# Wangshihu12/Voxel-SLAM

Measured on AMD Instinct MI355X. Metric: local-BA iterations/sec (200k pts, W=10), higher is better.
Workload: dtype f64

## Files before the change

### voxel-slam_amd/csrc/vba_kernels_li.hpp

```cpp
#pragma once
#include <hip/hip_runtime.h>
#include "vba_hostmath.hpp"
#include "vba_li_order.hpp"

namespace vba {

constexpr int LI_MAX_W = 16;
constexpr int LI_MAX_N = 15 * LI_MAX_W + 3;

struct LiDev {
  int W, n, nb, gravity, gauge, F;
  double imu_coef;
  double ex[LI_MAX_W * 12];
  double ext[LI_MAX_W * 12];
  double tstamp[LI_MAX_W];
  double rimu[2];
  double ext_spec[LM_SPEC][LI_MAX_W * 12];
  double ginc_spec[LM_SPEC][4];
  double binc_spec[LM_SPEC][LI_MAX_W * 6];
};

__device__ __forceinline__ void li_state(const double *pose12, const double *ex12, double t, vbh::State &s) {
  s.t = t;
#pragma unroll
// ... 332 lines not shown
  if (tid < F) {
    vbh::State s1, s2;
    li_state(s->xt + 12 * tid, li->ext + 12 * tid, li->tstamp[tid], s1);
    li_state(s->xt + 12 * (tid + 1), li->ext + 12 * (tid + 1), li->tstamp[tid + 1], s2);
    double rr[15];
    vbh::imu_residual_jacobian(*reinterpret_cast<const vbh::ImuPre *>(imu + 304 * (size_t)tid), s1, s2, li->gravity != 0, rr, nullptr, li->nb);
    for (int k = 0; k < 15; k++) rr_s[tid][k] = rr[k];
  }
  __syncthreads();
  if (tid < 15 * F) {
    const int f = tid / 15, r = tid - 15 * f;
    const double *m = imu + 304 * (size_t)f + 79 + 15 * r;
    double a = 0;
    for (int k = 0; k < 15; k++) a += m[k] * rr_s[f][k];
    a_s[f][r] = a;
  }
  __syncthreads();
  if (tid >= 64) return;
  double qi = 0.0;
  if (lane < F) for (int r = 0; r < 15; r++) qi += rr_s[lane][r] * a_s[lane][r];
  double rimu = 0.0;
  for (int f = 0; f < F; f++) rimu += readlane_f64(qi, f);
  double r2;
  if (nb > 0) {
    double acc = r2acc;
    for (int m = 32; m >= 1; m >>= 1) acc += __shfl_xor(acc, m, 64);
    r2 = acc;
  } else {
    r2 = readlane_f64(r2acc, 0);
  }
  r2 += rimu * (li->imu_coef * 0.5);
  const bool have_spec = spec_nx < spec_n;
  const int sc = have_spec ? spec_nx : 0;
  double q = r1 - r2, u = u0, v = v0;
  const bool accept = q > 0;
  if (accept) {
    for (int t = lane; t < 12 * W; t += 64) { s->x[t] = s->xt[t]; li->ex[t] = li->ext[t]; }
    const double one_three = 1.0 / 3;
    q = q / q1;
    v = 2;
    const double t = 2 * q - 1;
    q = 1 - t * t * t;
    u *= (q < one_three ? one_three : q);
  } else {
    u = u * v;
    v = 2 * v;
    if (lane < F) { double *m = imu + 304 * (size_t)lane; for (int k = 0; k < 3; k++) { m[67 + k] = m[73 + k]; m[70 + k] = m[76 + k]; } }
    if (have_spec) {
      double gn[3] = {0, 0, 0};
      if (li->gravity) for (int k = 0; k < 3; k++) gn[k] = li->ext[9 + k] + li->ginc_spec[sc][k];
      for (int t = lane; t < 12 * W; t += 64) {
        s->xt[t] = s->xt_spec[sc][t];
        const int k = t % 12;
        if (k < 9) li->ext[t] = li->ext_spec[sc][t];
        else if (li->gravity) li->ext[t] = gn[k - 9];
      }
      if (lane < F) {
        double *m = imu + 304 * (size_t)lane;
        for (int k = 0; k < 6; k++) m[67 + k] = m[73 + k] + li->binc_spec[sc][6 * lane + k];
      }
    }
  }
  if (lane != 0) return;
  if (!accept && have_spec) { s->q1 = s->q1_spec[sc]; s->spec_i = sc; s->use_spec = 1; }
  else { s->use_spec = 0; s->spec_n = 0; }
  li->rimu[1] = rimu;
  s->r2 = r2;
  if (ntr < mtr) {
    double *t = s->trace + 5 * ntr;
    t[0] = r1; t[1] = r2; t[2] = u0; t[3] = v0; t[4] = q1;
    s->n_trace = ntr + 1;
  }
  s->u = u; s->v = v;
  s->is_calc_hess = accept ? 1 : 0;
  s->last_accepted = accept ? 1 : 0;
  if (!accept) s->all_accepted = 0;
  s->iter = it + 1;
  const int nstop = (fabs((r1 - r2) / r1) < 1e-6) ? 1 : 0;
  s->stop = nstop;
  s->run_res = nstop ? 0 : 1;
  s->run_hess = (accept && !nstop) ? 1 : 0;
}

struct PackSegs { int n; const double *src[8]; size_t off[8], len[8]; };
__global__ void k_pack_segments(PackSegs p, double *__restrict__ dst) {
  const int s = blockIdx.y;
  if (s >= p.n) return;
  const double *src = p.src[s];
  double *d = dst + p.off[s];
  for (size_t i = (size_t)blockIdx.x * blockDim.x + threadIdx.x; i < p.len[s]; i += (size_t)gridDim.x * blockDim.x) d[i] = src[i];
}

}
```

### voxel-slam_amd/csrc/vba_li_order.hpp

```cpp
#pragma once

#if defined(__HIPCC__)
#include <hip/hip_runtime.h>
#define LIO_HD __host__ __device__ inline
#else
#define LIO_HD inline
#endif

namespace vba {

LIO_HD int li_ord(int k, int W) {
  if (k < 9 * W) { const int i = k / 9; return 15 * i + 6 + (k - 9 * i); }
  if (k < 15 * W) { const int q = k - 9 * W, i = q / 6; return 15 * i + (q - 6 * i); }
  return k;
}

LIO_HD unsigned li_live(int kb, int W, int n, int NP) {
  const int c0 = 8 * kb, c1 = c0 + 7;
  auto span = [](int a, int b) -> unsigned { return (a < b) ? ((2u << ((b - 1) >> 4)) - 1u) & ~((1u << (a >> 4)) - 1u) : 0u; };
  if (c0 >= 9 * W) return span(c0, NP);
  const int ihi = (c1 < 9 * W ? c1 : 9 * W - 1) / 9;
  unsigned m = span(c0, (9 * (ihi + 2) < 9 * W) ? 9 * (ihi + 2) : 9 * W);
  m |= span(9 * W, (6 * (ihi + 2) < 6 * W) ? 9 * W + 6 * (ihi + 2) : 15 * W);
  m |= span(15 * W, n + 1);
  if (c1 >= 9 * W) m |= span(9 * W, NP);
  return m;
}

LIO_HD int li_hb_pair(int a, int b) { return (3 * a + (b - a)) * 225; }
LIO_HD int li_hb_ne1(int W) { return (3 * W - 2) * 225; }
LIO_HD int li_hb_size(int W, int grav) { return li_hb_ne1(W) + (grav ? 90 * W + 9 : 0); }
LIO_HD double li_hb_get(const double *hb, int W, int n, int R, int C) {
  const int nw = 15 * W;
  if (R < nw && C < nw) { const int a = R / 15, b = C / 15; if (a - b > 1 || b - a > 1) return 0.0; return hb[li_hb_pair(a, b) + (R - 15 * a) * 15 + (C - 15 * b)]; }
  const int ne1 = li_hb_ne1(W);
  if (R < nw) return hb[ne1 + R * 3 + (C - nw)];
  if (C < nw) return hb[ne1 + 45 * W + (R - nw) * nw + C];
  return hb[ne1 + 90 * W + (R - nw) * 3 + (C - nw)];
}

}

#undef LIO_HD
```

### voxel-slam_amd/csrc/voxelba.hip

```cpp
#include "vba_ctx.hpp"
#include "vba_kernels_factor.hpp"
#include "vba_kernels_h3.hpp"
#include "vba_kernels_lm.hpp"
#include "vba_kernels_li.hpp"
#include <cstddef>
#include "vba_hostmath.hpp"

#include <hip/hip_runtime.h>
#include <rccl/rccl.h>
#include <dlfcn.h>
#include <cstdio>
#include <cstdlib>
#include <cstring>
#include <string>
#include <vector>
#include <array>
#include <map>
#include <chrono>
#include <algorithm>

using namespace vba;

namespace {

// ... 733 lines not shown
    return VBA_OK;
  }
  double *h_hess = nullptr;
  if (hess) {
    st = ensure_pin(c, 65536 + (size_t)n * n + 1024);
    if (st) return st;
    h_hess = c->h_pin + 32768;
  }
  const double *src = c->collective() ? c->d_raw : c->d_out;
  const int upd = c->lm.pending_update ? 1 : 0;
  switch (W) {
#define VBA_FIN_CASE(WW) case WW: hipLaunchKernelGGL(k_lm_finish<WW>, dim3(hess ? 17 : 1), dim3(256), 0, c->stream, c->d_lm, c->d_k4part, upd ? c->lm.k4_nb : 0, upd, c->h_lm, src, h_hess); break;
    VBA_FIN_CASE(2) VBA_FIN_CASE(3) VBA_FIN_CASE(4) VBA_FIN_CASE(5) VBA_FIN_CASE(6) VBA_FIN_CASE(7) VBA_FIN_CASE(8) VBA_FIN_CASE(9) VBA_FIN_CASE(10)
    VBA_FIN_CASE(11) VBA_FIN_CASE(12) VBA_FIN_CASE(13) VBA_FIN_CASE(14) VBA_FIN_CASE(15) VBA_FIN_CASE(16)
#undef VBA_FIN_CASE
    default: return VBA_ERR_UNSUPPORTED_WINDOW;
  }
  c->lm.pending_update = false;
  HIPCHK(c, hipGetLastError());
  HIPCHK(c, hipStreamSynchronize(c->stream));
  const LmDev *h = c->h_lm;
  if (poses) std::memcpy(poses, h->x, (size_t)W * 12 * sizeof(double));
  if (hess) std::memcpy(hess, c->h_pin + 32768, (size_t)n * n * sizeof(double));
  if (resis2) { resis2[0] = h->resis_first; resis2[1] = h->r2; }
  c->trace.assign(h->trace, h->trace + 5 * h->n_trace);
  if (h->pad & 16) {
    fprintf(stderr, "[k_lm_solve_m cycles] prologue %lld | tile load %lld | factorisation %lld | backsub %lld | epilogue %lld | panels:", h->stamps[1] - h->stamps[0],
            h->stamps[2] - h->stamps[1], h->stamps[3] - h->stamps[2], h->stamps[4] - h->stamps[3], h->stamps[5] - h->stamps[4]);
    const int npr = (int)h->stamps[6];
    for (int kb = 0; kb < npr && kb < 8; kb++) fprintf(stderr, " %lld+%lld", h->stamps[9 + 2 * kb] - h->stamps[8 + 2 * kb], kb < npr - 1 ? h->stamps[10 + 2 * kb] - h->stamps[9 + 2 * kb] : 0LL);
    fprintf(stderr, " | %d panels run\n", npr);
  }
  c->lm.active = false;
  return VBA_OK;
}

int vba_lidar_ba_damping_iter(vba_ctx *c, double *poses, double *hess, double *resis2, int max_iter, int thd_num, int *is_converge) {
  int st = vba_lm_begin(c, poses, thd_num);
  if (st) return st;
  for (int i = 0; i < max_iter; i++) {
    st = vba_lm_iterate(c, nullptr, nullptr);
    if (st) { c->lm.active = false; return st; }
  }
  st = vba_lm_end(c, poses, hess, resis2);
  if (is_converge) *is_converge = c->h_lm->all_accepted;
  return st;
}

int vba_last_lm_trace(vba_ctx *c, double *rows, int max_rows) {
  int n = (int)(c->trace.size() / 5);
  if (n > max_rows) n = max_rows;
  if (rows) std::memcpy(rows, c->trace.data(), (size_t)n * 5 * sizeof(double));
  return n;
}

extern "C++" {
template <int W>
struct LiSolveCfg {
  static constexpr int NMAX = 15 * W + 3, NP = ((NMAX + 1 + 15) / 16) * 16;
  static constexpr bool GL = W > 10;
  static constexpr size_t l_doubles = (size_t)LdltCfg<NP>::LTOT > (size_t)NMAX * (NMAX + 1) / 2 ? (size_t)LdltCfg<NP>::LTOT : (size_t)NMAX * (NMAX + 1) / 2;
  static constexpr size_t lds = ((GL ? (size_t)LdltCfg<NP>::DOUBLES - LdltCfg<NP>::LTOT : (size_t)LdltCfg<NP>::DOUBLES) + 4 * NMAX + NP + 32) * 8 + (size_t)NMAX * 4 + 64;
  static_assert(GL || l_doubles == (size_t)LdltCfg<NP>::LTOT, "the staged triangle must fit the region of L");
};
template <int W, int NT = (W > 10 ? 1024 : 512)>
static int launch_li_solve(vba_ctx *c, int copy_raw, int n, int gauge, int grav) {
  constexpr bool GL = LiSolveCfg<W>::GL;
  constexpr size_t l_doubles = LiSolveCfg<W>::l_doubles, lds = LiSolveCfg<W>::lds;
  static bool attr_set[kMaxDevices] = {false};
  if (!attr_set[c->device % kMaxDevices]) { hipFuncSetAttribute((const void *)k_li_solve<W, NT, GL>, hipFuncAttributeMaxDynamicSharedMemorySize, (int)lds); attr_set[c->device % kMaxDevices] = true; }
  if (GL && c->d_liscr.n < l_doubles * LM_SPEC) {
    HIPCHK(c, hipStreamSynchronize(c->stream));
    HIPCHK(c, c->d_liscr.ensure(l_doubles * LM_SPEC));
  }
  hipLaunchKernelGGL((k_li_solve<W, NT, GL>), dim3(c->lm_spec), dim3(NT), lds, c->stream, c->d_lm, c->d_li, c->d_out, c->d_raw, copy_raw, c->d_himu, c->d_gimu, c->d_imu, n, gauge, grav,
                     c->opt.imu_coef, c->d_liscr, nullptr);
  return VBA_OK;
}
namespace vba {
bool li_device_supported(int W) { return W >= 2 && W <= LI_MAX_W; }
}
}

static int li_setup(vba_ctx *c, const double *states, const double *imus, int gravity, LiDev &h, std::vector<double> &fimg) {
  const int W = c->opt.win_size, DIM = VBA_DIM, F = W - 1;
  const int n = W * DIM + (gravity ? 3 : 0), nb = gravity ? 33 : 30;
  if (!c->d_li) {
    HIPCHK(c, c->d_li.ensure(1));
    HIPCHK(c, c->d_imu.ensure((size_t)LI_MAX_W * 304));
    HIPCHK(c, c->d_himu.ensure((size_t)LI_MAX_N * LI_MAX_N));
    HIPCHK(c, c->d_gimu.ensure((size_t)LI_MAX_N));
  }
  std::vector<double> poses((size_t)W * 12);
  states_to_poses(states, W, poses.data());
  int st = vba_lm_begin(c, poses.data(), 0);
  if (st) return st;
  st = lm_init_flush(c);
  if (st) return st;
  h = LiDev{};
  h.W = W; h.n = n; h.nb = nb; h.gravity = gravity ? 1 : 0; h.gauge = gravity ? 6 : DIM; h.F = F; h.imu_coef = c->opt.imu_coef;
  for (int i = 0; i < W; i++) {
    const double *sx = states + 25 * i;
    h.tstamp[i] = sx[0];
    for (int k = 0; k < 12; k++) h.ex[12 * i + k] = h.ext[12 * i + k] = sx[13 + k];
  }
  fimg.resize((size_t)F * 304);
  std::memcpy(fimg.data(), imus, fimg.size() * sizeof(double));
  for (int f = 0; f < F; f++) {
    const double *cov = imus + 304 * (size_t)f + 79;
    double *dst = fimg.data() + 304 * (size_t)f + 79;
    bool hit = false;
    for (auto &e : c->covinv_cache)
      if (std::memcmp(e.data(), cov, 225 * sizeof(double)) == 0) { std::memcpy(dst, e.data() + 225, 225 * sizeof(double)); hit = true; break; }
    if (!hit) {
      vbh::inverse_pplu(cov, dst, 15);
      const bool grow = c->covinv_cache.size() < 32;
      if (grow) c->covinv_cache.emplace_back();
      auto &e = grow ? c->covinv_cache.back() : c->covinv_cache[c->covinv_next++ % 32];
      std::memcpy(e.data(), cov, 225 * sizeof(double)); std::memcpy(e.data() + 225, dst, 225 * sizeof(double));
    }
  }
  {
    HIPCHK(c, hipMemcpyAsync(c->d_li, &h, sizeof(LiDev), hipMemcpyHostToDevice, c->stream));
    HIPCHK(c, hipMemcpyAsync(c->d_imu, fimg.data(), fimg.size() * sizeof(double), hipMemcpyHostToDevice, c->stream));
  }
  HIPCHK(c, hipMemsetAsync(c->d_himu, 0, (size_t)li_hb_size(W, 1) * sizeof(double), c->stream));
  HIPCHK(c, hipMemsetAsync(c->d_gimu, 0, (size_t)n * sizeof(double), c->stream));
  {
    static bool attr_set[kMaxDevices] = {false};
    constexpr int FM = LI_MAX_W - 1;
    if (!attr_set[c->device % kMaxDevices]) { hipFuncSetAttribute((const void *)k_li_imu, hipFuncAttributeMaxDynamicSharedMemorySize, (int)(((size_t)2 * FM * 15 * 33 + 2 * FM * 15 + FM + 16) * sizeof(double))); attr_set[c->device % kMaxDevices] = true; }
  }
  return VBA_OK;
}
static size_t li_imu_lds(int F, int nb) { return ((size_t)2 * F * 15 * nb + 2 * F * 15 + F + 16) * sizeof(double); }
static bool li_imu_rides(const vba_ctx *c, int copy_raw, int V, size_t lds_imu) { return !(copy_raw && c->lm.have_hess) && V > 0 && lds_imu <= 150 * 1024; }

static int li_ba_device(vba_ctx *c, double *states, double *imus, int gravity, int max_iter, double *hess, double *resis2) {
  static const bool want_times = diag_env("VBA_LI_TIMES") != nullptr;
  const auto t_0 = std::chrono::steady_clock::now();
  auto since = [&](std::chrono::steady_clock::time_point a) { return std::chrono::duration<double, std::micro>(std::chrono::steady_clock::now() - a).count(); };
  const int W = c->opt.win_size, V = c->nvox, DIM = VBA_DIM, F = W - 1;
  const int n = W * DIM + (gravity ? 3 : 0), nb = gravity ? 33 : 30, n6 = 6 * W;
  if (!gravity) max_iter = 3;
  LiDev h{};
  std::vector<double> fimg;
  int st = li_setup(c, states, imus, gravity, h, fimg);
  if (st) return st;
  char *base = reinterpret_cast<char *>(c->d_lm.p);
  const double *x_dev = reinterpret_cast<const double *>(base + offsetof(LmDev, x));
  const double *xt_dev = reinterpret_cast<const double *>(base + offsetof(LmDev, xt));
  const int *run_hess = reinterpret_cast<const int *>(base + offsetof(LmDev, run_hess));
  const int *run_res = reinterpret_cast<const int *>(base + offsetof(LmDev, run_res));
  const int copy_raw = c->collective() ? 1 : 0;
  const size_t lds_imu = li_imu_lds(F, nb);
  const double t_up = since(t_0);
  for (int it = 0; it < max_iter; it++) {
    const bool lidar_now = li_imu_rides(c, copy_raw, V, lds_imu);
    if (lidar_now) {
      const LiJob job{c->d_lm, c->d_li, c->d_imu, c->d_himu, c->d_gimu};
      st = hessian_pass(c, x_dev, run_hess, 0, V, nullptr, nullptr, 0, job, lds_imu);
    } else {
      hipLaunchKernelGGL(k_li_imu, dim3(1), dim3(LI_IMU_NT), lds_imu, c->stream, c->d_lm, c->d_li, c->d_imu, c->d_himu, c->d_gimu);
      if (!(copy_raw && c->lm.have_hess)) st = hessian_pass(c, x_dev, run_hess, 0, V);
    }
    if (st) { c->lm.active = false; return st; }
    TimedSpan s1{};
    span_begin(c, "solve", s1);
    switch (W) {
      case 2: st = launch_li_solve<2>(c, copy_raw, n, h.gauge, h.gravity); break;
      case 3: st = launch_li_solve<3>(c, copy_raw, n, h.gauge, h.gravity); break;
      case 4: st = launch_li_solve<4>(c, copy_raw, n, h.gauge, h.gravity); break;
      case 5: st = launch_li_solve<5>(c, copy_raw, n, h.gauge, h.gravity); break;
      case 6: st = launch_li_solve<6>(c, copy_raw, n, h.gauge, h.gravity); break;
      case 7: st = launch_li_solve<7>(c, copy_raw, n, h.gauge, h.gravity); break;
      case 9: st = launch_li_solve<9>(c, copy_raw, n, h.gauge, h.gravity); break;
      case 8: st = launch_li_solve<8>(c, copy_raw, n, h.gauge, h.gravity); break;
      case 10: {
        static const int nt = diag_env("VBA_LI_NT") ? atoi(diag_env("VBA_LI_NT")) : 512;
        if (nt == 256) st = launch_li_solve<10, 256>(c, copy_raw, n, h.gauge, h.gravity); else if (nt == 1024) st = launch_li_solve<10, 1024>(c, copy_raw, n, h.gauge, h.gravity); else st = launch_li_solve<10, 512>(c, copy_raw, n, h.gauge, h.gravity);
        break;
      }
      case 11: st = launch_li_solve<11>(c, copy_raw, n, h.gauge, h.gravity); break;
      case 12: st = launch_li_solve<12>(c, copy_raw, n, h.gauge, h.gravity); break;
      case 13: st = launch_li_solve<13>(c, copy_raw, n, h.gauge, h.gravity); break;
      case 14: st = launch_li_solve<14>(c, copy_raw, n, h.gauge, h.gravity); break;
      case 15: st = launch_li_solve<15>(c, copy_raw, n, h.gauge, h.gravity); break;
      case 16: st = launch_li_solve<16>(c, copy_raw, n, h.gauge, h.gravity); break;
      default: c->lm.active = false; return VBA_ERR_UNSUPPORTED_WINDOW;
    }
    span_end(c, "solve", s1);
    if (st) { c->lm.active = false; return st; }
    if (copy_raw) {
      if (V > 0) launch_residual(c, xt_dev, run_res, 0, V);
      st = hessian_pass(c, xt_dev, run_res, 0, V);
      if (st) { c->lm.active = false; return st; }
      c->lm.have_hess = true;
      hipLaunchKernelGGL(k_li_update, dim3(1), dim3(LI_UPD_NT), 0, c->stream, c->d_lm, c->d_li, c->d_imu, c->d_out + (nout_tl(W) - 1), 0);
    } else if (V == 0) {
      st = residual_pass(c, xt_dev, run_res, 0, V, c->d_scal);
      if (st) { c->lm.active = false; return st; }
      hipLaunchKernelGGL(k_li_update, dim3(1), dim3(LI_UPD_NT), 0, c->stream, c->d_lm, c->d_li, c->d_imu, c->d_scal, 0);
    } else {
      const int nbk = residual_nb(c, V);
      TimedSpan s2{};
      span_begin(c, "residual", s2);
      launch_residual(c, xt_dev, run_res, 0, V);
      span_end(c, "residual", s2);
      hipLaunchKernelGGL(k_li_update, dim3(1), dim3(LI_UPD_NT), 0, c->stream, c->d_lm, c->d_li, c->d_imu, c->d_partial, nbk);
    }
    HIPCHK(c, hipGetLastError());
  }
  const double t_enq = since(t_0);
  const double t_gpu = since(t_0);
  static_assert(sizeof(LiDev) % 8 == 0 && sizeof(LmDev) % 8 == 0, "packed as doubles");
  const size_t o_li = 0, o_img = o_li + sizeof(LiDev) / 8, o_hb = o_img + fimg.size(), o_lid = o_hb + (size_t)li_hb_size(W, 1),
               o_lm = o_lid + (size_t)n6 * n6, o_end = o_lm + sizeof(LmDev) / 8;
  st = ensure_pin(c, o_end + 64);
  if (st) return st;
  HIPCHK(c, c->d_lipack.ensure(o_end + 64));
  PackSegs segs{};
  segs.n = 3;
  segs.src[0] = (const double *)c->d_li.p; segs.off[0] = o_li; segs.len[0] = sizeof(LiDev) / 8;
  segs.src[1] = c->d_imu; segs.off[1] = o_img; segs.len[1] = fimg.size();
  segs.src[2] = (const double *)c->d_lm.p; segs.off[2] = o_lm; segs.len[2] = sizeof(LmDev) / 8;
  if (hess) {
    st = tiles_to_full(c, copy_raw ? c->d_raw : c->d_out);
    if (st) return st;
    segs.n = 5;
    segs.src[3] = c->d_full; segs.off[3] = o_lid; segs.len[3] = (size_t)n6 * n6;
    segs.src[4] = c->d_himu; segs.off[4] = o_hb; segs.len[4] = (size_t)li_hb_size(W, gravity);
  }
  hipLaunchKernelGGL(k_pack_segments, dim3(64, segs.n), dim3(256), 0, c->stream, segs, c->d_lipack);
  HIPCHK(c, hipGetLastError());
  HIPCHK(c, hipMemcpyAsync(c->h_pin, c->d_lipack, o_end * sizeof(double), hipMemcpyDeviceToHost, c->stream));
  HIPCHK(c, hipStreamSynchronize(c->stream));
  std::memcpy(c->h_lm, c->h_pin + o_lm, sizeof(LmDev));
  std::memcpy(&h, c->h_pin + o_li, sizeof(LiDev));
  std::memcpy(fimg.data(), c->h_pin + o_img, fimg.size() * sizeof(double));
  const double *himu_h = c->h_pin + o_hb;
  c->lm.active = false;
  const LmDev *hl = c->h_lm;
  for (int i = 0; i < W; i++) {
    double *sx = states + 25 * i;
    for (int k = 0; k < 12; k++) sx[1 + k] = hl->x[12 * i + k];
    for (int k = 0; k < 12; k++) sx[13 + k] = h.ex[12 * i + k];
  }
  if (hl->use_spec)
    for (int f = 0; f < F; f++) std::memcpy(fimg.data() + 304 * (size_t)f + 67, fimg.data() + 304 * (size_t)f + 73, 6 * sizeof(double));
  for (int f = 0; f < F; f++) std::memcpy(imus + 304 * (size_t)f + 67, fimg.data() + 304 * (size_t)f + 67, 12 * sizeof(double));
  if (hess) {
    const double *lid = c->h_pin + o_lid;
    for (int r = 0; r < n; r++)
      for (int k = 0; k < n; k++) hess[(size_t)r * n + k] = c->opt.imu_coef * li_hb_get(himu_h, W, n, r, k);
    for (int i = 0; i < W; i++)
      for (int j = 0; j < W; j++)
        for (int r = 0; r < 6; r++)
          for (int k = 0; k < 6; k++) hess[(size_t)(i * DIM + r) * n + j * DIM + k] += lid[(size_t)(i * 6 + r) * n6 + j * 6 + k];
  }
  if (gravity && resis2) { resis2[0] = hl->resis_first; resis2[1] = hl->r2; }
  c->trace.assign(hl->trace, hl->trace + 5 * hl->n_trace);
  if (want_times && (hl->pad & 16)) {
    fprintf(stderr, "[k_li_solve prologue] stage imu %lld | stage lidar %lld | diag+g %lld | rank %lld\n", hl->stamps[50] - hl->stamps[0], hl->stamps[51] - hl->stamps[50], hl->stamps[52] - hl->stamps[51], hl->stamps[1] - hl->stamps[52]);
    fprintf(stderr, "[k_li_solve cycles] prologue %lld | tile load %lld | factorisation %lld | backsub %lld | epilogue %lld | panels:", hl->stamps[1] - hl->stamps[0],
            hl->stamps[2] - hl->stamps[1], hl->stamps[3] - hl->stamps[2], hl->stamps[4] - hl->stamps[3], hl->stamps[5] - hl->stamps[4]);
    const int npr = (int)hl->stamps[6];
    for (int kb = 0; kb < npr && kb < 20; kb++) fprintf(stderr, " %lld+%lld", hl->stamps[9 + 2 * kb] - hl->stamps[8 + 2 * kb], kb < npr - 1 ? hl->stamps[10 + 2 * kb] - hl->stamps[9 + 2 * kb] : 0LL);
    fprintf(stderr, " | %d panels run\n", npr);
  }
  if (want_times && (hl->pad & 64)) fprintf(stderr, "[k_li_imu cycles] factor algebra (one lane per factor) %lld | cov^-1 joc %lld | contractions %lld\n", hl->stamps[41] - hl->stamps[40], hl->stamps[42] - hl->stamps[41], hl->stamps[43] - hl->stamps[42]);
  if (want_times && (hl->pad & 32)) { double v[6]; std::memcpy(v, &hl->stamps[58], sizeof(v)); fprintf(stderr, "[li r1 parts] rank %d: rimu %.10g lidar %.10g | %.10g %.10g | %.10g %.10g\n", c->rank, v[0], v[1], v[2], v[3], v[4], v[5]); }
  if (want_times) fprintf(stderr, "[li_ba_device] upload %.1f us | enqueue %.1f | gpu drained at %.1f | total %.1f\n", t_up, t_enq - t_up, t_gpu, since(t_0));
  return VBA_OK;
}

int vba_li_ba_damping_iter(vba_ctx *c, double *states, double *imus, int gravity, int max_iter, double *hess, double *resis2) {
  if (!li_device_supported(c->opt.win_size)) return VBA_ERR_UNSUPPORTED_WINDOW;
  return li_ba_device(c, states, imus, gravity, max_iter, hess, resis2);
}

static int debug_li_imu_run(vba_ctx *c, int gravity, int flags, const double *states, const double *imus, double *h_dense, double *g, double *rimu,
                            double *covinv_out) {
  const int W = c->opt.win_size, V = c->nvox, F = W - 1, n = 15 * W + (gravity ? 3 : 0), nb = gravity ? 33 : 30;
  LiDev h{};
  std::vector<double> fimg;
  int st = li_setup(c, states, imus, gravity, h, fimg);
  if (st) return st;
  char *base = reinterpret_cast<char *>(c->d_lm.p);
  const double *x_dev = reinterpret_cast<const double *>(base + offsetof(LmDev, x));
  const int *run_hess = reinterpret_cast<const int *>(base + offsetof(LmDev, run_hess));
  const size_t lds_imu = li_imu_lds(F, nb);
  if (flags & (VBA_IMU_RIDE_H2 | VBA_IMU_RIDE_H3)) {
    const LiJob job{c->d_lm, c->d_li, c->d_imu, c->d_himu, c->d_gimu};
    st = hessian_pass(c, x_dev, run_hess, 0, V, nullptr, nullptr, 0, job, lds_imu);
    if (st) return st;
  } else {
    hipLaunchKernelGGL(k_li_imu, dim3(1), dim3(LI_IMU_NT), lds_imu, c->stream, c->d_lm, c->d_li, c->d_imu, c->d_himu, c->d_gimu);
  }
  HIPCHK(c, hipGetLastError());
  if (flags & VBA_IMU_TRIAL) {
    HIPCHK(c, hipMemsetAsync(c->d_scal, 0, sizeof(double), c->stream));
    hipLaunchKernelGGL(k_li_update, dim3(1), dim3(LI_UPD_NT), 0, c->stream, c->d_lm, c->d_li, c->d_imu, c->d_scal, 0);
    HIPCHK(c, hipGetLastError());
  }
  std::vector<double> hb((size_t)li_hb_size(W, gravity));
  hipError_t e = hipMemcpyAsync(hb.data(), c->d_himu, hb.size() * sizeof(double), hipMemcpyDeviceToHost, c->stream);
  if (e == hipSuccess) e = hipMemcpyAsync(g, c->d_gimu, (size_t)n * sizeof(double), hipMemcpyDeviceToHost, c->stream);
  if (e == hipSuccess) e = hipMemcpyAsync(&h, c->d_li, sizeof(LiDev), hipMemcpyDeviceToHost, c->stream);
  const hipError_t es = hipStreamSynchronize(c->stream);
  HIPCHK(c, e);
  HIPCHK(c, es);
  for (int r = 0; r < n; r++)
    for (int k = 0; k < n; k++) h_dense[(size_t)r * n + k] = li_hb_get(hb.data(), W, n, r, k);
  rimu[0] = h.rimu[0];
  rimu[1] = (flags & VBA_IMU_TRIAL) ? h.rimu[1] : 0.0;
  if (covinv_out)
    for (int f = 0; f < F; f++) std::memcpy(covinv_out + 225 * (size_t)f, fimg.data() + 304 * (size_t)f + 79, 225 * sizeof(double));
  return VBA_OK;
}
int vba_debug_li_imu(vba_ctx *c, int W, int gravity, int flags, const double *states, const double *imus, double *h_dense, double *g, double *rimu,
                     double *covinv_out) {
  if (!c || !states || !imus || !h_dense || !g || !rimu) return VBA_ERR_BAD_ARG;
  if (W != c->opt.win_size || !li_device_supported(W) || (gravity != 0 && gravity != 1)) return VBA_ERR_BAD_ARG;
  if (flags & ~(VBA_IMU_RIDE_H2 | VBA_IMU_RIDE_H3 | VBA_IMU_TRIAL)) return VBA_ERR_BAD_ARG;
  const bool h2 = (flags & VBA_IMU_RIDE_H2) != 0, h3 = (flags & VBA_IMU_RIDE_H3) != 0;
  if (h2 && h3) return VBA_ERR_BAD_ARG;
  if (c->collective()) return VBA_ERR_UNSUPPORTED;
  if (h2 || h3) {
    const bool ctx_h3 = c->use_h3 && W <= 10;
    if (c->nvox <= 0 || h3 != ctx_h3) return VBA_ERR_BAD_ARG;
    if (!li_imu_rides(c, 0, c->nvox, li_imu_lds(W - 1, gravity ? 33 : 30))) return VBA_ERR_BAD_ARG;
  }
  for (size_t i = 0; i < (size_t)25 * W; i++) if (!std::isfinite(states[i])) return VBA_ERR_BAD_ARG;
  for (size_t i = 0; i < (size_t)304 * (W - 1); i++) if (!std::isfinite(imus[i])) return VBA_ERR_BAD_ARG;
  HIPCHK(c, hipSetDevice(c->device));
  const int st = debug_li_imu_run(c, gravity, flags, states, imus, h_dense, g, rimu, covinv_out);
  if (st) hipStreamSynchronize(c->stream);
  c->lm_init.pending = false;
  c->lm.active = false;
  return st;
}

int vba_imu_preintegrate(int n, const double *t, const double *gyr, const double *acc, const double *bg, const double *ba,
                         const double *nm6, const double *nw6, double scale_gravity, double *out) {
  if (n < 1 || !t || !gyr || !acc || !out) return VBA_ERR_BAD_ARG;
  vbh::ImuPre m;
  vbh::imu_init(m, bg, ba);
  vbh::imu_push(m, n, t, gyr, acc, nm6, nw6, scale_gravity);
  std::memcpy(out, &m, sizeof(m));
  return VBA_OK;
}
int vba_imu_give_evaluate(const double *imu_pre, const double *s1, const double *s2, int with_gravity, int jac_enable, double *jtj,
                          double *gg, double *resid) {
  if (!imu_pre || !s1 || !s2) return VBA_ERR_BAD_ARG;
  const double r = vbh::imu_evaluate(*reinterpret_cast<const vbh::ImuPre *>(imu_pre), *reinterpret_cast<const vbh::State *>(s1),
                                     *reinterpret_cast<const vbh::State *>(s2), with_gravity != 0, jac_enable != 0, jtj, gg);
  if (resid) *resid = r;
  return VBA_OK;
}

int vba_set_allreduce(vba_ctx *c, vba_allreduce_fn fn, void *user) { c->allreduce = fn; c->allreduce_user = user; return VBA_OK; }

int vba_rccl_get_unique_id(void *out128) {
  if (!out128) return VBA_ERR_BAD_ARG;
  static_assert(sizeof(ncclUniqueId) == 128, "ncclUniqueId is 128 bytes");
  const RcclApi &R = rccl_api();
  if (!R.ok) return VBA_ERR_UNSUPPORTED;
  ncclUniqueId id;
  if (R.GetUniqueId(&id) != ncclSuccess) return VBA_ERR_HIP;
  std::memcpy(out128, &id, sizeof(id));
  return VBA_OK;
}
int vba_rccl_init(vba_ctx *c, const void *unique_id128, int rank, int n_ranks) {
  if (!c || !unique_id128 || n_ranks < 1 || rank < 0 || rank >= n_ranks) return VBA_ERR_BAD_ARG;
  const RcclApi &R = rccl_api();
  if (!R.ok) { c->set_error(R.why); return VBA_ERR_UNSUPPORTED; }
  if (c->comm && c->own_comm) { R.CommDestroy(c->comm); c->comm = nullptr; }
  ncclUniqueId id;
  std::memcpy(&id, unique_id128, sizeof(id));
  HIPCHK(c, hipSetDevice(c->device));
  const ncclResult_t r = R.CommInitRank(&c->comm, n_ranks, id, rank);
  if (r != ncclSuccess) { c->comm = nullptr; c->set_error(std::string("ncclCommInitRank: ") + R.GetErrorString(r)); return VBA_ERR_HIP; }
  c->own_comm = true;
  return vba_set_shard(c, rank, n_ranks);
}
int vba_set_rccl_comm(vba_ctx *c, void *nccl_comm) {
  if (!c) return VBA_ERR_BAD_ARG;
  const RcclApi &R = rccl_api();
  if (!R.ok) { c->set_error(R.why); return VBA_ERR_UNSUPPORTED; }
  if (c->comm && c->own_comm) R.CommDestroy(c->comm);
  c->comm = (ncclComm_t)nccl_comm; c->own_comm = false;
  return VBA_OK;
}
int vba_shard_owner(int64_t kx, int64_t ky, int64_t kz, int n_ranks) {
  if (n_ranks <= 1) return 0;
  return (int)(vba::shard_bucket(kx, ky, kz) * (uint64_t)n_ranks >> 16);
}
int vba_set_shard(vba_ctx *c, int rank, int n_ranks) {
  if (n_ranks < 1 || rank < 0 || rank >= n_ranks) return VBA_ERR_BAD_ARG;
  c->rank = rank; c->n_ranks = n_ranks;
// ... 275 lines not shown
```

Baseline: 22990.

## Fuse LI setup into init kernel and pack only needed results on finish

Replaces the separate host-built LiDev upload, memsets and lm_init_flush with one k_li_init kernel that takes its parameters as kernel arguments. It stages the factor image in pinned memory instead of a pageable vector. At the end, k_li_finish gathers only the needed LmDev head, extrinsics, factor biases, IMU Hessian blocks and tile-expanded Hessian into a single compact readback. This drops the separate tiles_to_full pass and most of the full-struct copies. Hessian assembly on the host now uses direct block copies instead of a per-element getter. The cost is a larger kernarg payload, a per-window template switch and a fixed pinned-buffer layout limit.

```diff
diff --git a/voxel-slam_amd/csrc/vba_kernels_li.hpp b/voxel-slam_amd/csrc/vba_kernels_li.hpp
--- a/voxel-slam_amd/csrc/vba_kernels_li.hpp
+++ b/voxel-slam_amd/csrc/vba_kernels_li.hpp
@@ -438,13 +438,72 @@
   s->run_hess = (accept && !nstop) ? 1 : 0;
 }
 
-struct PackSegs { int n; const double *src[8]; size_t off[8], len[8]; };
-__global__ void k_pack_segments(PackSegs p, double *__restrict__ dst) {
-  const int s = blockIdx.y;
-  if (s >= p.n) return;
-  const double *src = p.src[s];
-  double *d = dst + p.off[s];
-  for (size_t i = (size_t)blockIdx.x * blockDim.x + threadIdx.x; i < p.len[s]; i += (size_t)gridDim.x * blockDim.x) d[i] = src[i];
-}
-
-}
+template <int W>
+struct LiInit {
+  int n, nb, gravity, gauge, F, nh;
+  double imu_coef;
+  double tstamp[W];
+  double ex[12 * W];
+  LiDev *dst;
+  double *himu, *gimu;
+};
+static_assert(sizeof(LmInit<LI_MAX_W>) + sizeof(LiInit<LI_MAX_W>) <= 4096, "k_li_init's arguments stay within the 4 KB kernarg segment");
+constexpr int LI_INIT_NB = 8;
+template <int W>
+__global__ __launch_bounds__(256) void k_li_init(LmInit<W> lm, LiInit<W> a) {
+  constexpr int NW = sizeof(LiDev) / 8, EX = offsetof(LiDev, ex) / 8, EXT = offsetof(LiDev, ext) / 8, TS = offsetof(LiDev, tstamp) / 8;
+  static_assert(sizeof(LiDev) % 8 == 0 && offsetof(LiDev, W) == 0 && offsetof(LiDev, F) == 20 && offsetof(LiDev, imu_coef) == 24 && offsetof(LiDev, ex) == 32,
+                "the header is three words of two ints and imu_coef");
+  const int tid = threadIdx.x;
+  if (blockIdx.x == 0) {
+    lm_init_store(lm, tid, 256);
+    auto two = [](int lo, int hi) { return (unsigned long long)(unsigned int)lo | ((unsigned long long)(unsigned int)hi << 32); };
+    unsigned long long *o = reinterpret_cast<unsigned long long *>(a.dst);
+    for (int w = tid; w < NW; w += 256) {
+      unsigned long long val = 0ull;
+      if (w == 0) val = two(W, a.n);
+      else if (w == 1) val = two(a.nb, a.gravity);
+      else if (w == 2) val = two(a.gauge, a.F);
+      else if (w == 3) val = (unsigned long long)__double_as_longlong(a.imu_coef);
+      else if (w >= EX && w < EX + 12 * W) val = (unsigned long long)__double_as_longlong(a.ex[w - EX]);
+      else if (w >= EXT && w < EXT + 12 * W) val = (unsigned long long)__double_as_longlong(a.ex[w - EXT]);
+      else if (w >= TS && w < TS + W) val = (unsigned long long)__double_as_longlong(a.tstamp[w - TS]);
+      o[w] = val;
+    }
+  }
+  const int gt = blockIdx.x * 256 + tid, gn = gridDim.x * 256;
+  for (int t = gt; t < a.nh; t += gn) a.himu[t] = 0.0;
+  for (int t = gt; t < a.n; t += gn) a.gimu[t] = 0.0;
+}
+
+struct LiPack { int n_lm, o_ex, o_f, o_hb, o_lid, end; };
+inline LiPack li_pack_layout(int W, int gravity, bool hess) {
+  LiPack p{};
+  p.n_lm = (int)(offsetof(LmDev, q1_spec) / 8);
+  p.o_ex = p.n_lm; p.o_f = p.o_ex + 12 * W; p.o_hb = p.o_f + 12 * (W - 1);
+  p.o_lid = p.o_hb + (hess ? li_hb_size(W, gravity) : 0);
+  p.end = p.o_lid + (hess ? 36 * W * W : 0);
+  return p;
+}
+constexpr int LI_FIN_NB = 32;
+template <int W>
+__global__ __launch_bounds__(256) void k_li_finish(const LmDev *s, const LiDev *li, const double *__restrict__ imu, const double *__restrict__ himu,
+                                                   const double *__restrict__ red, double *__restrict__ dst, LiPack p) {
+  static_assert(offsetof(LmDev, q1_spec) % 8 == 0, "the head of LmDev is whole words");
+  const int use_spec = s->use_spec;
+  const double *lm = reinterpret_cast<const double *>(s);
+  for (int t = blockIdx.x * 256 + threadIdx.x; t < p.end; t += gridDim.x * 256) {
+    double v;
+    if (t < p.o_ex) v = lm[t];
+    else if (t < p.o_f) v = li->ex[t - p.o_ex];
+    else if (t < p.o_hb) {
+      const int q = t - p.o_f, f = q / 12, k = q - 12 * f;
+      v = imu[304 * (size_t)f + ((use_spec && k < 6) ? 73 + k : 67 + k)];
+    }
+    else if (t < p.o_lid) v = himu[t - p.o_hb];
+    else { const int e = t - p.o_lid, row = e / (6 * W); v = tl_fetch<W>(red, row, e - row * (6 * W)); }
+    dst[t] = v;
+  }
+}
+
+}
diff --git a/voxel-slam_amd/csrc/vba_li_order.hpp b/voxel-slam_amd/csrc/vba_li_order.hpp
--- a/voxel-slam_amd/csrc/vba_li_order.hpp
+++ b/voxel-slam_amd/csrc/vba_li_order.hpp
@@ -39,6 +39,34 @@
   return hb[ne1 + 90 * W + (R - nw) * 3 + (C - nw)];
 }
 
+LIO_HD void li_hess_assemble(double *hess, const double *hb, const double *lid, int W, int grav, double coef) {
+  const int nw = 15 * W, n = nw + (grav ? 3 : 0), n6 = 6 * W, ne1 = li_hb_ne1(W);
+  const double z = coef * 0.0;
+  for (long long e = 0; e < (long long)n * n; e++) hess[e] = z;
+  for (int a = 0; a < W; a++)
+    for (int b = (a > 0 ? a - 1 : 0); b <= a + 1 && b < W; b++) {
+      const double *src = hb + li_hb_pair(a, b);
+      double *dst = hess + (long long)(15 * a) * n + 15 * b;
+      for (int r = 0; r < 15; r++)
+        for (int k = 0; k < 15; k++) dst[(long long)r * n + k] = coef * src[15 * r + k];
+    }
+  if (grav) {
+    for (int R = 0; R < nw; R++)
+      for (int k = 0; k < 3; k++) hess[(long long)R * n + nw + k] = coef * hb[ne1 + R * 3 + k];
+    for (int k = 0; k < 3; k++)
+      for (int C = 0; C < nw; C++) hess[(long long)(nw + k) * n + C] = coef * hb[ne1 + 45 * W + k * nw + C];
+    for (int r = 0; r < 3; r++)
+      for (int k = 0; k < 3; k++) hess[(long long)(nw + r) * n + nw + k] = coef * hb[ne1 + 90 * W + 3 * r + k];
+  }
+  for (int i = 0; i < W; i++)
+    for (int j = 0; j < W; j++) {
+      const double *src = lid + (long long)(6 * i) * n6 + 6 * j;
+      double *dst = hess + (long long)(15 * i) * n + 15 * j;
+      for (int r = 0; r < 6; r++)
+        for (int k = 0; k < 6; k++) dst[(long long)r * n + k] += src[r * n6 + k];
+    }
+}
+
 }
 
 #undef LIO_HD
diff --git a/voxel-slam_amd/csrc/voxelba.hip b/voxel-slam_amd/csrc/voxelba.hip
--- a/voxel-slam_amd/csrc/voxelba.hip
+++ b/voxel-slam_amd/csrc/voxelba.hip
@@ -839,33 +839,43 @@
 }
 }
 
-static int li_setup(vba_ctx *c, const double *states, const double *imus, int gravity, LiDev &h, std::vector<double> &fimg) {
-  const int W = c->opt.win_size, DIM = VBA_DIM, F = W - 1;
-  const int n = W * DIM + (gravity ? 3 : 0), nb = gravity ? 33 : 30;
+constexpr size_t LI_PIN_UP = 32768, LI_PIN_DOUBLES = 65536;
+static_assert(LI_PIN_UP + (size_t)(LI_MAX_W - 1) * 304 <= 60000, "the factor image ends below the slot vba_lm_begin uses on a sharded rank");
+extern "C++" {
+template <int W>
+static void launch_li_init(vba_ctx *c, const double *states, int gravity) {
+  LiInit<W> a{};
+  a.n = W * VBA_DIM + (gravity ? 3 : 0); a.nb = gravity ? 33 : 30; a.gravity = gravity ? 1 : 0; a.gauge = gravity ? 6 : VBA_DIM; a.F = W - 1;
+  a.nh = li_hb_size(W, 1); a.imu_coef = c->opt.imu_coef;
+  for (int i = 0; i < W; i++) {
+    const double *sx = states + 25 * i;
+    a.tstamp[i] = sx[0];
+    for (int k = 0; k < 12; k++) a.ex[12 * i + k] = sx[13 + k];
+  }
+  a.dst = c->d_li; a.himu = c->d_himu; a.gimu = c->d_gimu;
+  hipLaunchKernelGGL(k_li_init<W>, dim3(LI_INIT_NB), dim3(256), 0, c->stream, lm_init_arg<W>(c, true), a);
+}
+}
+static int li_setup(vba_ctx *c, const double *states, const double *imus, int gravity) {
+  const int W = c->opt.win_size, F = W - 1;
   if (!c->d_li) {
     HIPCHK(c, c->d_li.ensure(1));
     HIPCHK(c, c->d_imu.ensure((size_t)LI_MAX_W * 304));
     HIPCHK(c, c->d_himu.ensure((size_t)LI_MAX_N * LI_MAX_N));
     HIPCHK(c, c->d_gimu.ensure((size_t)LI_MAX_N));
   }
+  int st = ensure_pin(c, LI_PIN_DOUBLES);
+  if (st) return st;
   std::vector<double> poses((size_t)W * 12);
   states_to_poses(states, W, poses.data());
-  int st = vba_lm_begin(c, poses.data(), 0);
-  if (st) return st;
-  st = lm_init_flush(c);
-  if (st) return st;
-  h = LiDev{};
-  h.W = W; h.n = n; h.nb = nb; h.gravity = gravity ? 1 : 0; h.gauge = gravity ? 6 : DIM; h.F = F; h.imu_coef = c->opt.imu_coef;
-  for (int i = 0; i < W; i++) {
-    const double *sx = states + 25 * i;
-    h.tstamp[i] = sx[0];
-    for (int k = 0; k < 12; k++) h.ex[12 * i + k] = h.ext[12 * i + k] = sx[13 + k];
-  }
-  fimg.resize((size_t)F * 304);
-  std::memcpy(fimg.data(), imus, fimg.size() * sizeof(double));
+  st = vba_lm_begin(c, poses.data(), 0);
+  if (st) return st;
+  double *fimg = c->h_pin + LI_PIN_UP;
+  const size_t nimg = (size_t)F * 304;
+  std::memcpy(fimg, imus, nimg * sizeof(double));
   for (int f = 0; f < F; f++) {
     const double *cov = imus + 304 * (size_t)f + 79;
-    double *dst = fimg.data() + 304 * (size_t)f + 79;
+    double *dst = fimg + 304 * (size_t)f + 79;
     bool hit = false;
     for (auto &e : c->covinv_cache)
       if (std::memcmp(e.data(), cov, 225 * sizeof(double)) == 0) { std::memcpy(dst, e.data() + 225, 225 * sizeof(double)); hit = true; break; }
@@ -877,12 +887,15 @@
       std::memcpy(e.data(), cov, 225 * sizeof(double)); std::memcpy(e.data() + 225, dst, 225 * sizeof(double));
     }
   }
-  {
-    HIPCHK(c, hipMemcpyAsync(c->d_li, &h, sizeof(LiDev), hipMemcpyHostToDevice, c->stream));
-    HIPCHK(c, hipMemcpyAsync(c->d_imu, fimg.data(), fimg.size() * sizeof(double), hipMemcpyHostToDevice, c->stream));
-  }
-  HIPCHK(c, hipMemsetAsync(c->d_himu, 0, (size_t)li_hb_size(W, 1) * sizeof(double), c->stream));
-  HIPCHK(c, hipMemsetAsync(c->d_gimu, 0, (size_t)n * sizeof(double), c->stream));
+  HIPCHK(c, hipMemcpyAsync(c->d_imu, fimg, nimg * sizeof(double), hipMemcpyHostToDevice, c->stream));
+  switch (W) {
+#define VBA_LII_CASE(WW) case WW: launch_li_init<WW>(c, states, gravity); break;
+    VBA_LII_CASE(2) VBA_LII_CASE(3) VBA_LII_CASE(4) VBA_LII_CASE(5) VBA_LII_CASE(6) VBA_LII_CASE(7) VBA_LII_CASE(8) VBA_LII_CASE(9) VBA_LII_CASE(10)
+    VBA_LII_CASE(11) VBA_LII_CASE(12) VBA_LII_CASE(13) VBA_LII_CASE(14) VBA_LII_CASE(15) VBA_LII_CASE(16)
+#undef VBA_LII_CASE
+    default: return VBA_ERR_UNSUPPORTED_WINDOW;
+  }
+  HIPCHK(c, hipGetLastError());
   {
     static bool attr_set[kMaxDevices] = {false};
     constexpr int FM = LI_MAX_W - 1;
@@ -900,9 +913,8 @@
   const int W = c->opt.win_size, V = c->nvox, DIM = VBA_DIM, F = W - 1;
   const int n = W * DIM + (gravity ? 3 : 0), nb = gravity ? 33 : 30, n6 = 6 * W;
   if (!gravity) max_iter = 3;
-  LiDev h{};
-  std::vector<double> fimg;
-  int st = li_setup(c, states, imus, gravity, h, fimg);
+  const int gauge = gravity ? 6 : DIM, grav = gravity ? 1 : 0;
+  int st = li_setup(c, states, imus, gravity);
   if (st) return st;
   char *base = reinterpret_cast<char *>(c->d_lm.p);
   const double *x_dev = reinterpret_cast<const double *>(base + offsetof(LmDev, x));
@@ -925,25 +937,25 @@
     TimedSpan s1{};
     span_begin(c, "solve", s1);
     switch (W) {
-      case 2: st = launch_li_solve<2>(c, copy_raw, n, h.gauge, h.gravity); break;
-      case 3: st = launch_li_solve<3>(c, copy_raw, n, h.gauge, h.gravity); break;
-      case 4: st = launch_li_solve<4>(c, copy_raw, n, h.gauge, h.gravity); break;
-      case 5: st = launch_li_solve<5>(c, copy_raw, n, h.gauge, h.gravity); break;
-      case 6: st = launch_li_solve<6>(c, copy_raw, n, h.gauge, h.gravity); break;
-      case 7: st = launch_li_solve<7>(c, copy_raw, n, h.gauge, h.gravity); break;
-      case 9: st = launch_li_solve<9>(c, copy_raw, n, h.gauge, h.gravity); break;
-      case 8: st = launch_li_solve<8>(c, copy_raw, n, h.gauge, h.gravity); break;
+      case 2: st = launch_li_solve<2>(c, copy_raw, n, gauge, grav); break;
+      case 3: st = launch_li_solve<3>(c, copy_raw, n, gauge, grav); break;
+      case 4: st = launch_li_solve<4>(c, copy_raw, n, gauge, grav); break;
+      case 5: st = launch_li_solve<5>(c, copy_raw, n, gauge, grav); break;
+      case 6: st = launch_li_solve<6>(c, copy_raw, n, gauge, grav); break;
+      case 7: st = launch_li_solve<7>(c, copy_raw, n, gauge, grav); break;
+      case 9: st = launch_li_solve<9>(c, copy_raw, n, gauge, grav); break;
+      case 8: st = launch_li_solve<8>(c, copy_raw, n, gauge, grav); break;
       case 10: {
         static const int nt = diag_env("VBA_LI_NT") ? atoi(diag_env("VBA_LI_NT")) : 512;
-        if (nt == 256) st = launch_li_solve<10, 256>(c, copy_raw, n, h.gauge, h.gravity); else if (nt == 1024) st = launch_li_solve<10, 1024>(c, copy_raw, n, h.gauge, h.gravity); else st = launch_li_solve<10, 512>(c, copy_raw, n, h.gauge, h.gravity);
+        if (nt == 256) st = launch_li_solve<10, 256>(c, copy_raw, n, gauge, grav); else if (nt == 1024) st = launch_li_solve<10, 1024>(c, copy_raw, n, gauge, grav); else st = launch_li_solve<10, 512>(c, copy_raw, n, gauge, grav);
         break;
       }
-      case 11: st = launch_li_solve<11>(c, copy_raw, n, h.gauge, h.gravity); break;
-      case 12: st = launch_li_solve<12>(c, copy_raw, n, h.gauge, h.gravity); break;
-      case 13: st = launch_li_solve<13>(c, copy_raw, n, h.gauge, h.gravity); break;
-      case 14: st = launch_li_solve<14>(c, copy_raw, n, h.gauge, h.gravity); break;
-      case 15: st = launch_li_solve<15>(c, copy_raw, n, h.gauge, h.gravity); break;
-      case 16: st = launch_li_solve<16>(c, copy_raw, n, h.gauge, h.gravity); break;
+      case 11: st = launch_li_solve<11>(c, copy_raw, n, gauge, grav); break;
+      case 12: st = launch_li_solve<12>(c, copy_raw, n, gauge, grav); break;
+      case 13: st = launch_li_solve<13>(c, copy_raw, n, gauge, grav); break;
+      case 14: st = launch_li_solve<14>(c, copy_raw, n, gauge, grav); break;
+      case 15: st = launch_li_solve<15>(c, copy_raw, n, gauge, grav); break;
+      case 16: st = launch_li_solve<16>(c, copy_raw, n, gauge, grav); break;
       default: c->lm.active = false; return VBA_ERR_UNSUPPORTED_WINDOW;
     }
     span_end(c, "solve", s1);
@@ -970,51 +982,33 @@
   }
   const double t_enq = since(t_0);
   const double t_gpu = since(t_0);
-  static_assert(sizeof(LiDev) % 8 == 0 && sizeof(LmDev) % 8 == 0, "packed as doubles");
-  const size_t o_li = 0, o_img = o_li + sizeof(LiDev) / 8, o_hb = o_img + fimg.size(), o_lid = o_hb + (size_t)li_hb_size(W, 1),
-               o_lm = o_lid + (size_t)n6 * n6, o_end = o_lm + sizeof(LmDev) / 8;
-  st = ensure_pin(c, o_end + 64);
-  if (st) return st;
-  HIPCHK(c, c->d_lipack.ensure(o_end + 64));
-  PackSegs segs{};
-  segs.n = 3;
-  segs.src[0] = (const double *)c->d_li.p; segs.off[0] = o_li; segs.len[0] = sizeof(LiDev) / 8;
-  segs.src[1] = c->d_imu; segs.off[1] = o_img; segs.len[1] = fimg.size();
-  segs.src[2] = (const double *)c->d_lm.p; segs.off[2] = o_lm; segs.len[2] = sizeof(LmDev) / 8;
-  if (hess) {
-    st = tiles_to_full(c, copy_raw ? c->d_raw : c->d_out);
-    if (st) return st;
-    segs.n = 5;
-    segs.src[3] = c->d_full; segs.off[3] = o_lid; segs.len[3] = (size_t)n6 * n6;
-    segs.src[4] = c->d_himu; segs.off[4] = o_hb; segs.len[4] = (size_t)li_hb_size(W, gravity);
-  }
-  hipLaunchKernelGGL(k_pack_segments, dim3(64, segs.n), dim3(256), 0, c->stream, segs, c->d_lipack);
+  const LiPack pk = li_pack_layout(W, gravity, hess != nullptr);
+  if ((size_t)pk.end > LI_PIN_UP) { c->lm.active = false; return VBA_ERR_UNSUPPORTED_WINDOW; }
+  HIPCHK(c, c->d_lipack.ensure((size_t)pk.end + 64));
+  {
+    const double *red = copy_raw ? c->d_raw : c->d_out;
+    switch (W) {
+#define VBA_LIF_CASE(WW) case WW: hipLaunchKernelGGL(k_li_finish<WW>, dim3(LI_FIN_NB), dim3(256), 0, c->stream, c->d_lm, c->d_li, c->d_imu, c->d_himu, red, c->d_lipack, pk); break;
+      VBA_LIF_CASE(2) VBA_LIF_CASE(3) VBA_LIF_CASE(4) VBA_LIF_CASE(5) VBA_LIF_CASE(6) VBA_LIF_CASE(7) VBA_LIF_CASE(8) VBA_LIF_CASE(9) VBA_LIF_CASE(10)
+      VBA_LIF_CASE(11) VBA_LIF_CASE(12) VBA_LIF_CASE(13) VBA_LIF_CASE(14) VBA_LIF_CASE(15) VBA_LIF_CASE(16)
+#undef VBA_LIF_CASE
+      default: c->lm.active = false; return VBA_ERR_UNSUPPORTED_WINDOW;
+    }
+  }
   HIPCHK(c, hipGetLastError());
-  HIPCHK(c, hipMemcpyAsync(c->h_pin, c->d_lipack, o_end * sizeof(double), hipMemcpyDeviceToHost, c->stream));
+  HIPCHK(c, hipMemcpyAsync(c->h_pin, c->d_lipack, (size_t)pk.end * sizeof(double), hipMemcpyDeviceToHost, c->stream));
   HIPCHK(c, hipStreamSynchronize(c->stream));
-  std::memcpy(c->h_lm, c->h_pin + o_lm, sizeof(LmDev));
-  std::memcpy(&h, c->h_pin + o_li, sizeof(LiDev));
-  std::memcpy(fimg.data(), c->h_pin + o_img, fimg.size() * sizeof(double));
-  const double *himu_h = c->h_pin + o_hb;
+  std::memcpy(c->h_lm, c->h_pin, (size_t)pk.n_lm * sizeof(double));
   c->lm.active = false;
   const LmDev *hl = c->h_lm;
+  const double *ex_h = c->h_pin + pk.o_ex, *fac_h = c->h_pin + pk.o_f;
   for (int i = 0; i < W; i++) {
     double *sx = states + 25 * i;
     for (int k = 0; k < 12; k++) sx[1 + k] = hl->x[12 * i + k];
-    for (int k = 0; k < 12; k++) sx[13 + k] = h.ex[12 * i + k];
-  }
-  if (hl->use_spec)
-    for (int f = 0; f < F; f++) std::memcpy(fimg.data() + 304 * (size_t)f + 67, fimg.data() + 304 * (size_t)f + 73, 6 * sizeof(double));
-  for (int f = 0; f < F; f++) std::memcpy(imus + 304 * (size_t)f + 67, fimg.data() + 304 * (size_t)f + 67, 12 * sizeof(double));
-  if (hess) {
-    const double *lid = c->h_pin + o_lid;
-    for (int r = 0; r < n; r++)
-      for (int k = 0; k < n; k++) hess[(size_t)r * n + k] = c->opt.imu_coef * li_hb_get(himu_h, W, n, r, k);
-    for (int i = 0; i < W; i++)
-      for (int j = 0; j < W; j++)
-        for (int r = 0; r < 6; r++)
-          for (int k = 0; k < 6; k++) hess[(size_t)(i * DIM + r) * n + j * DIM + k] += lid[(size_t)(i * 6 + r) * n6 + j * 6 + k];
-  }
+    for (int k = 0; k < 12; k++) sx[13 + k] = ex_h[12 * i + k];
+  }
+  for (int f = 0; f < F; f++) std::memcpy(imus + 304 * (size_t)f + 67, fac_h + 12 * (size_t)f, 12 * sizeof(double));
+  if (hess) li_hess_assemble(hess, c->h_pin + pk.o_hb, c->h_pin + pk.o_lid, W, grav, c->opt.imu_coef);
   if (gravity && resis2) { resis2[0] = hl->resis_first; resis2[1] = hl->r2; }
   c->trace.assign(hl->trace, hl->trace + 5 * hl->n_trace);
   if (want_times && (hl->pad & 16)) {
@@ -1040,9 +1034,9 @@
                             double *covinv_out) {
   const int W = c->opt.win_size, V = c->nvox, F = W - 1, n = 15 * W + (gravity ? 3 : 0), nb = gravity ? 33 : 30;
   LiDev h{};
-  std::vector<double> fimg;
-  int st = li_setup(c, states, imus, gravity, h, fimg);
-  if (st) return st;
+  int st = li_setup(c, states, imus, gravity);
+  if (st) return st;
+  const double *fimg = c->h_pin + LI_PIN_UP;
   char *base = reinterpret_cast<char *>(c->d_lm.p);
   const double *x_dev = reinterpret_cast<const double *>(base + offsetof(LmDev, x));
   const int *run_hess = reinterpret_cast<const int *>(base + offsetof(LmDev, run_hess));
@@ -1072,7 +1066,7 @@
   rimu[0] = h.rimu[0];
   rimu[1] = (flags & VBA_IMU_TRIAL) ? h.rimu[1] : 0.0;
   if (covinv_out)
-    for (int f = 0; f < F; f++) std::memcpy(covinv_out + 225 * (size_t)f, fimg.data() + 304 * (size_t)f + 79, 225 * sizeof(double));
+    for (int f = 0; f < F; f++) std::memcpy(covinv_out + 225 * (size_t)f, fimg + 304 * (size_t)f + 79, 225 * sizeof(double));
   return VBA_OK;
 }
 int vba_debug_li_imu(vba_ctx *c, int W, int gravity, int flags, const double *states, const double *imus, double *h_dense, double *g, double *rimu,
```

Result: no change. 23010, median of 2 (+0.1%).
